# facebookresearch/dpr-scale

Hardware: NVIDIA H100
Metric: query+ctx pairs/sec (BERT-base, seq128) (higher is better)
Workload: dtype bf16

## Files before the change

dpr_scale_b200/csrc/gemm_wgmma.cu:

```cuda
#include <cstdlib>
#include <vector>
#include "common.cuh"
#include "dprb_internal.h"

namespace dprb {

namespace {

constexpr int BLOCK_M = 128;
constexpr int BLOCK_N = 256;
constexpr int BLOCK_K = 64;
constexpr int STAGES = 3;
constexpr int A_TILE_BYTES = BLOCK_M * BLOCK_K * 2;
constexpr int B_TILE_BYTES = BLOCK_N * BLOCK_K * 2;
constexpr int STAGE_BYTES = A_TILE_BYTES + B_TILE_BYTES;
constexpr int NUM_CONSUMERS = 2;
constexpr int NUM_THREADS = (NUM_CONSUMERS + 1) * 128;
constexpr int WG_ROWS = BLOCK_M / NUM_CONSUMERS;
constexpr int SUB_COLS = 64;
constexpr int SUB_BYTES = WG_ROWS * SUB_COLS * 2;
constexpr int STG_BYTES = WG_ROWS * BLOCK_N * 2;
constexpr int SMEM_BYTES = STAGES * STAGE_BYTES + NUM_CONSUMERS * STG_BYTES + 1024  + 128 ;
static_assert(SMEM_BYTES <= 227 * 1024, "ring + staging must fit one CTA per SM");
constexpr int PRODUCER_REGS = 40, CONSUMER_REGS = 232;
static_assert(128 * PRODUCER_REGS + NUM_CONSUMERS * 128 * CONSUMER_REGS <= 65536, "register file");

struct GemmParams {
  int M, N, K;
  int num_m_blocks, num_n_blocks;
  int k_blocks_total, k_blocks_per_split, splits;
  int units;
  int epilogue;
  void* D;
  long long ldd;
  const float* bias;
  int has_aux;
  int has_out2;
  float alpha;
  float* colsum;
  Drop drop;
  int aux_f16, out_f16;
  int save_pre;
};

struct Unit {
  int m0, n0, kb0, kb1;
};
__device__ __forceinline__ Unit unit_at(const GemmParams& p, int u) {
  const int tiles = p.num_m_blocks * p.num_n_blocks;
  const int tile = u % tiles, split = u / tiles;
  Unit w;
  w.m0 = (tile / p.num_n_blocks) * BLOCK_M;
  w.n0 = (tile % p.num_n_blocks) * BLOCK_N;
  w.kb0 = split * p.k_blocks_per_split;
  w.kb1 = min(w.kb0 + p.k_blocks_per_split, p.k_blocks_total);
  return w;
}

__device__ __forceinline__ void red_add_v2_f32(float* p, float a, float b) {
  asm volatile("red.global.add.v2.f32 [%0], {%1, %2};" ::"l"(p), "f"(a), "f"(b) : "memory");
}
__device__ __forceinline__ void wg_bar(int wg) { asm volatile("bar.sync %0, 128;" ::"r"(wg + 1) : "memory"); }

template <int A_MN, int B_MN, int F16>
__device__ __forceinline__ void mma_kblock(float (&acc)[128], uint32_t sa, uint32_t sb, int accumulate_first) {
  const uint64_t da = make_wgmma_desc_sw128(sa, A_MN ? BLOCK_K * 128 : 16, 1024);
  const uint64_t db = make_wgmma_desc_sw128(sb, B_MN ? BLOCK_K * 128 : 16, 1024);
  constexpr uint32_t A_KSTEP = (A_MN ? 16 * 128 : 32) >> 4;
  constexpr uint32_t B_KSTEP = (B_MN ? 16 * 128 : 32) >> 4;
#pragma unroll
  for (int k = 0; k < BLOCK_K / 16; ++k) {
    const int accum = (k > 0 || accumulate_first) ? 1 : 0;
    if (F16) wgmma_m64n256_ss_f16<A_MN, B_MN>(acc, da + k * A_KSTEP, db + k * B_KSTEP, accum);
    else wgmma_m64n256_ss_bf16<A_MN, B_MN>(acc, da + k * A_KSTEP, db + k * B_KSTEP, accum);
  }
}

__device__ __forceinline__ uint32_t pack_out(float a, float b, bool f16) { return f16 ? pack_f16x2(a, b) : pack_bf16x2(a, b); }

__device__ __forceinline__ uint32_t slab_base(const uint8_t* stg, int lr, int q) {
  return smem_u32(stg) + lr * 128 + ((lr & 7) << 4) + 4 * q;
}
__device__ __forceinline__ uint32_t slab_pair(uint32_t base, int c, int h) {
  return (base ^ ((c & 7) << 4)) + (c >> 3) * SUB_BYTES + h * 8 * 128;
}
__device__ __forceinline__ void sts32(uint32_t a, uint32_t v) { asm volatile("st.shared.b32 [%0], %1;" ::"r"(a), "r"(v)); }
__device__ __forceinline__ uint32_t lds32(uint32_t a) {
  uint32_t v;
  asm volatile("ld.shared.b32 %0, [%1];" : "=r"(v) : "r"(a));
  return v;
}
__device__ __forceinline__ int slab_boxes(int row0, int n0, int M, int N) {
  return row0 < M ? min(BLOCK_N / SUB_COLS, (N - n0 + SUB_COLS - 1) / SUB_COLS) : 0;
}
__device__ __forceinline__ void slab_tma_store(const CUtensorMap* m, const uint8_t* stg, int row0, int n0, int M, int N) {
  const int boxes = slab_boxes(row0, n0, M, N);
  for (int s = 0; s < boxes; ++s) tma_store_2d(m, smem_u32(stg + s * SUB_BYTES), n0 + s * SUB_COLS, row0);
  tma_store_commit();
}

template <bool ATOMIC>
__device__ __forceinline__ void epilogue_f32(const GemmParams& p, const float (&acc)[128], int row0, int n0, int lr, int q) {
#pragma unroll
  for (int h = 0; h < 2; ++h) {
    const int row = row0 + lr + 8 * h;
    if (row >= p.M) continue;
    float* drow = reinterpret_cast<float*>(p.D) + (long long)row * p.ldd;
#pragma unroll
    for (int c = 0; c < 32; ++c) {
      const int col = n0 + 8 * c + 2 * q;
      const float x = acc[4 * c + 2 * h] * p.alpha, y = acc[4 * c + 2 * h + 1] * p.alpha;
      if (ATOMIC) {
        if (col + 1 < p.N) red_add_v2_f32(drow + col, x, y);
        else if (col < p.N) atomicAdd(drow + col, x);
      } else {
        if (col < p.N) drow[col] = x + (p.bias != nullptr ? __ldg(p.bias + col) : 0.f);
        if (col + 1 < p.N) drow[col + 1] = y + (p.bias != nullptr ? __ldg(p.bias + col + 1) : 0.f);
      }
    }
  }
}

template <int EP, bool DROP, bool COLSUM>
__device__ __forceinline__ void epilogue16(const GemmParams& p, float (&acc)[128], uint32_t slab, int row0, int n0, int lr,
                                           int q, int lane) {
  const bool out_f16 = p.out_f16 != 0, aux_f16 = p.aux_f16 != 0;
#pragma unroll
  for (int c = 0; c < 32; ++c) {
    const int col = n0 + 8 * c + 2 * q;
    float2 b = make_float2(0.f, 0.f);
    if (p.bias != nullptr) {
      if (col + 1 < p.N) b = __ldg(reinterpret_cast<const float2*>(p.bias + col));
      else if (col < p.N) b.x = __ldg(p.bias + col);
    }
    float cs0 = 0.f, cs1 = 0.f;
#pragma unroll
    for (int h = 0; h < 2; ++h) {
      const int row = row0 + lr + 8 * h;
      const uint32_t sp = slab_pair(slab, c, h);
      float2 v = ffma2(make_float2(acc[4 * c + 2 * h], acc[4 * c + 2 * h + 1]), make_float2(p.alpha, p.alpha), b);
      if constexpr (EP == DPRB_EPI_BIAS_GELU) {
        float2 g, d;
        gelu_and_grad2(v, g, d);
        if (p.save_pre) d = v;
        sts32(sp, pack_bf16x2(g.x, g.y));
        acc[4 * c + 2 * h] = d.x;
        acc[4 * c + 2 * h + 1] = d.y;
        continue;
      }
      if constexpr (DROP) {
        float m0f, m1f;
        p.drop.mul2((uint32_t)row, (uint32_t)col, m0f, m1f);
        v.x *= m0f; v.y *= m1f;
      }
      if constexpr (EP == DPRB_EPI_BIAS_RESIDUAL) {
        const float2 a = unpack_16x2(lds32(sp), aux_f16);
        v.x += a.x; v.y += a.y;
      } else if constexpr (EP == DPRB_EPI_DGELU) {
        const float2 a = unpack_bf16x2(lds32(sp));
        v.x *= a.x; v.y *= a.y;
      } else if constexpr (EP == DPRB_EPI_DGELU_PRE) {
        float2 g, d;
        gelu_and_grad2(unpack_bf16x2(lds32(sp)), g, d);
        v.x *= d.x; v.y *= d.y;
      }
      const uint32_t o = pack_out(v.x, v.y, out_f16);
      sts32(sp, o);
      if (COLSUM && row < p.M && col < p.N) {
        const float2 f = unpack_bf16x2(o);
        cs0 += f.x;
        if (col + 1 < p.N) cs1 += f.y;
      }
    }
    if (COLSUM) {
#pragma unroll
      for (int o = 4; o < 32; o <<= 1) {
        cs0 += __shfl_xor_sync(0xFFFFFFFFu, cs0, o);
        cs1 += __shfl_xor_sync(0xFFFFFFFFu, cs1, o);
      }
      if (lane < 4) {
        if (col < p.N) atomicAdd(p.colsum + col, cs0);
        if (col + 1 < p.N) atomicAdd(p.colsum + col + 1, cs1);
      }
    }
  }
}

template <int A_MN, int B_MN, int F16>
__global__ void __launch_bounds__(NUM_THREADS, 1)
gemm_bf16_kernel(const __grid_constant__ CUtensorMap tmap_a, const __grid_constant__ CUtensorMap tmap_b,
                 const __grid_constant__ CUtensorMap tmap_d, const __grid_constant__ CUtensorMap tmap_aux,
                 const __grid_constant__ CUtensorMap tmap_out2, const GemmParams p) {
  extern __shared__ uint8_t smem_raw[];
  uint8_t* smem = align1024(smem_raw);
  uint8_t* staging = smem + STAGES * STAGE_BYTES;
  uint64_t* full_bar = reinterpret_cast<uint64_t*>(staging + NUM_CONSUMERS * STG_BYTES);
  uint64_t* empty_bar = full_bar + STAGES;
  uint64_t* aux_full = empty_bar + STAGES;
  uint64_t* slab_empty = aux_full + NUM_CONSUMERS;

  const int warp = threadIdx.x >> 5;
  const int lane = threadIdx.x & 31;
  const bool out16 = p.epilogue != DPRB_EPI_F32_ATOMIC_ADD && p.epilogue != DPRB_EPI_F32_STORE;

  if (threadIdx.x == 0) {
    tma_prefetch_desc(&tmap_a);
    tma_prefetch_desc(&tmap_b);
    if (out16) tma_prefetch_desc(&tmap_d);
    if (p.has_aux) tma_prefetch_desc(&tmap_aux);
    if (p.has_out2) tma_prefetch_desc(&tmap_out2);
    for (int i = 0; i < STAGES; ++i) {
      mbar_init(&full_bar[i], 1);
      mbar_init(&empty_bar[i], NUM_CONSUMERS * 4);
    }
    for (int i = 0; i < NUM_CONSUMERS; ++i) {
      mbar_init(&aux_full[i], 1);
      mbar_init(&slab_empty[i], 1);
    }
    fence_barrier_init();
  }
  __syncthreads();

  if (warp < 4) {
    asm volatile("setmaxnreg.dec.sync.aligned.u32 %0;" ::"n"(PRODUCER_REGS));
    if (warp == 0 && lane == 0) {
      int stage = 0;
      uint32_t phase = 0, uphase = 0;
      for (int u = blockIdx.x; u < p.units; u += gridDim.x, uphase ^= 1) {
        const Unit w = unit_at(p, u);
        const int aux_kb = min(w.kb0 + 2, w.kb1 - 1);
        for (int kb = w.kb0; kb < w.kb1; ++kb) {
          mbar_wait(&empty_bar[stage], phase ^ 1);
          mbar_arrive_expect_tx(&full_bar[stage], STAGE_BYTES);
          uint8_t* sa = smem + stage * STAGE_BYTES;
          uint8_t* sb = sa + A_TILE_BYTES;
          if (A_MN == 0) {
            tma_load_2d(sa, &tmap_a, &full_bar[stage], kb * BLOCK_K, w.m0);
          } else {
#pragma unroll
            for (int i = 0; i < BLOCK_M / 64; ++i) tma_load_2d(sa + i * (BLOCK_K * 128), &tmap_a, &full_bar[stage], w.m0 + i * 64, kb * BLOCK_K);
          }
          if (B_MN == 0) {
            tma_load_2d(sb, &tmap_b, &full_bar[stage], kb * BLOCK_K, w.n0);
          } else {
#pragma unroll
            for (int i = 0; i < BLOCK_N / 64; ++i) tma_load_2d(sb + i * (BLOCK_K * 128), &tmap_b, &full_bar[stage], w.n0 + i * 64, kb * BLOCK_K);
          }
          if (++stage == STAGES) { stage = 0; phase ^= 1; }
          if (p.has_aux && kb == aux_kb) {
            for (int g = 0; g < NUM_CONSUMERS; ++g) {
              const int row0 = w.m0 + g * WG_ROWS;
              const int boxes = slab_boxes(row0, w.n0, p.M, p.N);
              uint8_t* slab = staging + g * STG_BYTES;
              mbar_wait(&slab_empty[g], uphase);
              mbar_arrive_expect_tx(&aux_full[g], boxes * SUB_BYTES);
              for (int s = 0; s < boxes; ++s)
                tma_load_2d(slab + s * SUB_BYTES, &tmap_aux, &aux_full[g], w.n0 + s * SUB_COLS, row0);
            }
          }
        }
      }
    }
    return;
  }

  asm volatile("setmaxnreg.inc.sync.aligned.u32 %0;" ::"n"(CONSUMER_REGS));
  const int wg = (warp >> 2) - 1;
  const int t = threadIdx.x - 128 * (wg + 1);
  uint8_t* stg = staging + wg * STG_BYTES;
  const uint32_t a_off = (uint32_t)wg * (A_MN ? BLOCK_K * 128 : 64 * 128);
  const int q = lane & 3;
  const int lr = (warp & 3) * 16 + (lane >> 2);
  const uint32_t slab = slab_base(stg, lr, q);
  const int ep = p.epilogue;

  float acc[128];
  int stage = 0;
  uint32_t phase = 0, uphase = 0;
  for (int u = blockIdx.x; u < p.units; u += gridDim.x, uphase ^= 1) {
    const Unit w = unit_at(p, u);
    {
      int prev = -1;
      const int release_kb = min(w.kb0 + 1, w.kb1 - 1);
      for (int kb = w.kb0; kb < w.kb1; ++kb) {
        mbar_wait(&full_bar[stage], phase);
        const uint32_t sa = smem_u32(smem + stage * STAGE_BYTES) + a_off;
        const uint32_t sb = smem_u32(smem + stage * STAGE_BYTES + A_TILE_BYTES);
        wgmma_fence();
        mma_kblock<A_MN, B_MN, F16>(acc, sa, sb, kb > w.kb0);
        wgmma_commit();
        wgmma_wait<1>();
        if (prev >= 0) {
          __syncwarp();
          if (lane == 0) mbar_arrive(&empty_bar[prev]);
        }
        if (p.has_aux && kb == release_kb && t == 0) {
          tma_store_wait_read();
          mbar_arrive(&slab_empty[wg]);
        }
        prev = stage;
        if (++stage == STAGES) { stage = 0; phase ^= 1; }
      }
      wgmma_wait<0>();
      __syncwarp();
      if (lane == 0) mbar_arrive(&empty_bar[prev]);
    }

    const int row0 = w.m0 + wg * WG_ROWS;
    switch (ep) {
      case DPRB_EPI_F32_ATOMIC_ADD: epilogue_f32<true>(p, acc, row0, w.n0, lr, q); continue;
      case DPRB_EPI_F32_STORE: epilogue_f32<false>(p, acc, row0, w.n0, lr, q); continue;
      default: break;
    }
    if (p.has_aux) mbar_wait(&aux_full[wg], uphase);
    else if (t == 0) tma_store_wait_read();
    wg_bar(wg);
    const bool cs = p.colsum != nullptr, drop = p.drop.on();
    switch (ep) {
      case DPRB_EPI_BIAS:
        if (cs) epilogue16<DPRB_EPI_BIAS, false, true>(p, acc, slab, row0, w.n0, lr, q, lane);
        else epilogue16<DPRB_EPI_BIAS, false, false>(p, acc, slab, row0, w.n0, lr, q, lane);
        break;
      case DPRB_EPI_BIAS_GELU: epilogue16<DPRB_EPI_BIAS_GELU, false, false>(p, acc, slab, row0, w.n0, lr, q, lane); break;
      case DPRB_EPI_BIAS_RESIDUAL:
        if (drop) {
          if (cs) epilogue16<DPRB_EPI_BIAS_RESIDUAL, true, true>(p, acc, slab, row0, w.n0, lr, q, lane);
          else epilogue16<DPRB_EPI_BIAS_RESIDUAL, true, false>(p, acc, slab, row0, w.n0, lr, q, lane);
        } else {
          if (cs) epilogue16<DPRB_EPI_BIAS_RESIDUAL, false, true>(p, acc, slab, row0, w.n0, lr, q, lane);
          else epilogue16<DPRB_EPI_BIAS_RESIDUAL, false, false>(p, acc, slab, row0, w.n0, lr, q, lane);
        }
        break;
      case DPRB_EPI_DGELU:
        if (cs) epilogue16<DPRB_EPI_DGELU, false, true>(p, acc, slab, row0, w.n0, lr, q, lane);
        else epilogue16<DPRB_EPI_DGELU, false, false>(p, acc, slab, row0, w.n0, lr, q, lane);
        break;
      default:
        if (cs) epilogue16<DPRB_EPI_DGELU_PRE, false, true>(p, acc, slab, row0, w.n0, lr, q, lane);
        else epilogue16<DPRB_EPI_DGELU_PRE, false, false>(p, acc, slab, row0, w.n0, lr, q, lane);
        break;
    }
    fence_proxy_async_smem();
    wg_bar(wg);
    if (t == 0) slab_tma_store(&tmap_d, stg, row0, w.n0, p.M, p.N);
    if (p.has_out2) {
      if (t == 0) tma_store_wait_read();
      wg_bar(wg);
#pragma unroll
      for (int c = 0; c < 32; ++c)
#pragma unroll
        for (int h = 0; h < 2; ++h)
          sts32(slab_pair(slab, c, h), pack_bf16x2(acc[4 * c + 2 * h], acc[4 * c + 2 * h + 1]));
      fence_proxy_async_smem();
      wg_bar(wg);
      if (t == 0) slab_tma_store(&tmap_out2, stg, row0, w.n0, p.M, p.N);
    }
  }
  if (t == 0) tma_store_wait_all();
}

int make_tmap(CUtensorMap* out, const void* base, long long rows, long long cols, long long ld, int box_rows) {
  DPRB_REQUIRE((reinterpret_cast<uintptr_t>(base) & 15) == 0, "gemm operand base %p not 16-byte aligned", base);
  DPRB_REQUIRE((ld * 2) % 16 == 0, "gemm operand leading dimension %lld not a multiple of 8 elements", ld);
  const cuuint64_t dims[2] = {(cuuint64_t)cols, (cuuint64_t)rows};
  const cuuint64_t strides[1] = {(cuuint64_t)ld * 2};
  const cuuint32_t box[2] = {64u, (cuuint32_t)box_rows};
  return encode_tmap(out, "gemm", CU_TENSOR_MAP_DATA_TYPE_BFLOAT16, 2, base, dims, strides, box,
                     CU_TENSOR_MAP_L2_PROMOTION_L2_256B);
}

struct GemmProfile {
  bool enabled = false;
  std::vector<cudaEvent_t> ev;
  std::vector<double> flops;
  size_t used = 0;
};
GemmProfile g_prof;

int choose_splits(int tiles, int k_blocks, int sms) {
  int best = 1;
  double best_cost = 1e30;
  for (int s = 1; s <= 32; ++s) {
    if (k_blocks / s < 4 && s > 1) break;
    const int rounds = (tiles * s + sms - 1) / sms;
    const double cost = (double)rounds * ((k_blocks + s - 1) / s + 4);
    if (cost < best_cost - 1e-9) { best_cost = cost; best = s; }
  }
  return best;
}

}

int gemm_bf16(const void* A, const void* B, void* D, int M, int N, int K, long long lda, long long ldb,
              long long ldd, int a_mn_major, int b_mn_major, int epilogue, const float* bias, const void* aux,
              long long ld_aux, void* out2, float alpha, int splits, float* colsum, float dropout_p,
              unsigned long long drop_site_seed, cudaStream_t stream) {
  DPRB_REQUIRE(M > 0 && N > 0 && K > 0, "gemm: empty problem M=%d N=%d K=%d", M, N, K);
  const int dt_flags = epilogue & ~0xFF;
  epilogue &= 0xFF;
  const int a_f16 = (dt_flags & DPRB_GEMM_A_F16) != 0, b_f16 = (dt_flags & DPRB_GEMM_B_F16) != 0;
  const int aux_f16 = (dt_flags & DPRB_GEMM_AUX_F16) != 0, out_f16 = (dt_flags & DPRB_GEMM_OUT_F16) != 0;
  DPRB_REQUIRE(epilogue >= 0 && epilogue < DPRB_EPI_COUNT, "gemm: bad epilogue %d", epilogue);
  DPRB_REQUIRE(!(aux_f16 || out_f16) || epilogue == DPRB_EPI_BIAS || epilogue == DPRB_EPI_BIAS_RESIDUAL,
               "gemm: fp16 aux / output is implemented for the BIAS and BIAS_RESIDUAL epilogues only");
  DPRB_REQUIRE(a_f16 == b_f16, "gemm: wgmma takes no fp16 x bf16 operand pair: give "
               "DPRB_GEMM_A_F16 and DPRB_GEMM_B_F16 together or not at all");
  DPRB_REQUIRE(!out_f16 || colsum == nullptr, "gemm: colsum reads a bf16 slab (not available with fp16 output)");
  const bool f32_out = (epilogue == DPRB_EPI_F32_ATOMIC_ADD || epilogue == DPRB_EPI_F32_STORE);
  DPRB_REQUIRE(f32_out || (ldd % 8 == 0 && (reinterpret_cast<uintptr_t>(D) & 15) == 0),
               "gemm: bf16 output must be 16-byte aligned with ldd %% 8 == 0 (ldd=%lld)", ldd);
  DPRB_REQUIRE(!f32_out || (ldd % 4 == 0 && (reinterpret_cast<uintptr_t>(D) & 15) == 0),
               "gemm: fp32 output must be 16-byte aligned with ldd %% 4 == 0 (ldd=%lld)", ldd);
  const bool has_aux = epilogue == DPRB_EPI_BIAS_RESIDUAL || epilogue == DPRB_EPI_DGELU || epilogue == DPRB_EPI_DGELU_PRE;
  if (has_aux)
    DPRB_REQUIRE(aux != nullptr && ld_aux % 8 == 0 && (reinterpret_cast<uintptr_t>(aux) & 15) == 0,
                 "gemm: epilogue %d needs a 16-byte aligned aux with ld %% 8 == 0", epilogue);
  if (bias != nullptr) DPRB_REQUIRE((reinterpret_cast<uintptr_t>(bias) & 15) == 0, "gemm: bias not 16B aligned");

  DPRB_REQUIRE(colsum == nullptr || (!f32_out && epilogue != DPRB_EPI_BIAS_GELU),
               "gemm: colsum is supported for the BIAS / BIAS_RESIDUAL / DGELU epilogues only");

  const bool has_out2 = epilogue == DPRB_EPI_BIAS_GELU && out2 != nullptr;
  if (has_out2)
    DPRB_REQUIRE((reinterpret_cast<uintptr_t>(out2) & 15) == 0, "gemm: out2 not 16-byte aligned");

  CUtensorMap ta, tb, td{}, tx{}, to2{};
  int rc;
  if (!a_mn_major) rc = make_tmap(&ta, A, M, K, lda, BLOCK_M); else rc = make_tmap(&ta, A, K, M, lda, BLOCK_K);
  if (rc) return rc;
  if (!b_mn_major) rc = make_tmap(&tb, B, N, K, ldb, BLOCK_N); else rc = make_tmap(&tb, B, K, N, ldb, BLOCK_K);
  if (rc) return rc;
  if (!f32_out && (rc = make_tmap(&td, D, M, N, ldd, WG_ROWS))) return rc;
  if (has_aux && (rc = make_tmap(&tx, aux, M, N, ld_aux, WG_ROWS))) return rc;
  if (has_out2 && (rc = make_tmap(&to2, out2, M, N, ldd, WG_ROWS))) return rc;

  GemmParams p;
  p.M = M; p.N = N; p.K = K;
  p.num_m_blocks = (M + BLOCK_M - 1) / BLOCK_M;
  p.num_n_blocks = (N + BLOCK_N - 1) / BLOCK_N;
  p.k_blocks_total = (K + BLOCK_K - 1) / BLOCK_K;
  DPRB_NUM_SMS(sms);
  const int tiles = p.num_m_blocks * p.num_n_blocks;
  if (epilogue != DPRB_EPI_F32_ATOMIC_ADD) splits = 1;
  else if (splits <= 0) splits = choose_splits(tiles, p.k_blocks_total, sms);
  if (splits > p.k_blocks_total) splits = p.k_blocks_total;
  p.k_blocks_per_split = (p.k_blocks_total + splits - 1) / splits;
  p.splits = (p.k_blocks_total + p.k_blocks_per_split - 1) / p.k_blocks_per_split;
  p.epilogue = epilogue;
  p.D = D; p.ldd = ldd; p.bias = bias; p.has_aux = has_aux; p.has_out2 = has_out2; p.alpha = alpha;
  p.colsum = colsum;
  p.aux_f16 = aux_f16; p.out_f16 = out_f16;
  p.save_pre = (dt_flags & DPRB_GEMM_SAVE_PRE) != 0;
  p.drop = drop_from_site(epilogue == DPRB_EPI_BIAS_RESIDUAL ? dropout_p : 0.f, drop_site_seed);

  p.units = tiles * p.splits;
  const int grid = p.units < sms ? p.units : sms;
  static bool attr_set = false;
  if (!attr_set) {
#define DPRB_SET_ATTR(...) DPRB_CHECK_CUDA(cudaFuncSetAttribute(__VA_ARGS__, cudaFuncAttributeMaxDynamicSharedMemorySize, SMEM_BYTES));
    DPRB_SET_ATTR(gemm_bf16_kernel<0, 0, 0>) DPRB_SET_ATTR(gemm_bf16_kernel<0, 1, 0>)
    DPRB_SET_ATTR(gemm_bf16_kernel<1, 0, 0>) DPRB_SET_ATTR(gemm_bf16_kernel<1, 1, 0>)
    DPRB_SET_ATTR(gemm_bf16_kernel<0, 0, 1>) DPRB_SET_ATTR(gemm_bf16_kernel<0, 1, 1>)
    DPRB_SET_ATTR(gemm_bf16_kernel<1, 0, 1>) DPRB_SET_ATTR(gemm_bf16_kernel<1, 1, 1>)
#undef DPRB_SET_ATTR
    attr_set = true;
  }
  auto launch = [&](auto kern) -> int {
    const bool prof = g_prof.enabled && g_prof.used + 2 <= g_prof.ev.size();
    if (prof) DPRB_CHECK_CUDA(cudaEventRecord(g_prof.ev[g_prof.used], stream));
    kern<<<grid, NUM_THREADS, SMEM_BYTES, stream>>>(ta, tb, td, tx, to2, p);
    DPRB_LAUNCH_CHECK();
    if (prof) {
      DPRB_CHECK_CUDA(cudaEventRecord(g_prof.ev[g_prof.used + 1], stream));
      g_prof.flops.push_back(2.0 * (double)M * (double)N * (double)K);
      g_prof.used += 2;
    }
    return 0;
  };
  const int key = (a_mn_major ? 4 : 0) | (b_mn_major ? 2 : 0) | (a_f16 ? 1 : 0);
  switch (key) {
    case 0: return launch(gemm_bf16_kernel<0, 0, 0>);
    case 1: return launch(gemm_bf16_kernel<0, 0, 1>);
    case 2: return launch(gemm_bf16_kernel<0, 1, 0>);
    case 3: return launch(gemm_bf16_kernel<0, 1, 1>);
    case 4: return launch(gemm_bf16_kernel<1, 0, 0>);
    case 5: return launch(gemm_bf16_kernel<1, 0, 1>);
    case 6: return launch(gemm_bf16_kernel<1, 1, 0>);
    default: return launch(gemm_bf16_kernel<1, 1, 1>);
  }
}

int gemm_profile_enable(int enable, int max_launches) {
  if (enable) {
    const size_t want = (size_t)max_launches * 2;
    while (g_prof.ev.size() < want) {
      cudaEvent_t e;
      DPRB_CHECK_CUDA(cudaEventCreate(&e));
      g_prof.ev.push_back(e);
    }
    g_prof.used = 0;
    g_prof.flops.clear();
  }
  g_prof.enabled = enable != 0;
  return 0;
}

int gemm_profile_read(double* total_ms, double* total_flops, long long* launches) {
  double ms = 0.0, fl = 0.0;
  for (size_t i = 0; i + 1 < g_prof.used; i += 2) {
    DPRB_CHECK_CUDA(cudaEventSynchronize(g_prof.ev[i + 1]));
    float t = 0.f;
    DPRB_CHECK_CUDA(cudaEventElapsedTime(&t, g_prof.ev[i], g_prof.ev[i + 1]));
    ms += t;
    fl += g_prof.flops[i / 2];
  }
  if (total_ms) *total_ms = ms;
  if (total_flops) *total_flops = fl;
  if (launches) *launches = (long long)(g_prof.used / 2);
  return 0;
}

}
```

Baseline: 764.1.

## Add ping-pong warpgroup GEMM kernel for short-K bf16-output GEMMs

Adds a ping-pong schedule GEMM in which the two consumer warpgroups each own a whole 128x128 tile and alternate mainloops through named barriers. This lets one warpgroup's epilogue overlap the other's MMA. It uses a 5-stage ring and prefetches the residual aux tile by TMA during the mainloop, and is selected for non-fp32 outputs with K up to 1024. The dropout-residual math is also fused into an FMA, with a rounding split between row halves. In exchange it uses narrower N tiles, which means more B reloads, and adds more synchronisation complexity.

Result: faster. 781.4 (median of 6 runs) (+2.3%).

```diff
diff --git a/dpr_scale_b200/csrc/gemm_pingpong_sched.h b/dpr_scale_b200/csrc/gemm_pingpong_sched.h
--- /dev/null
+++ b/dpr_scale_b200/csrc/gemm_pingpong_sched.h
@@ -0,0 +1,43 @@
+#pragma once
+
+#if defined(__CUDACC__)
+#define DPRB_HD __host__ __device__ __forceinline__
+#else
+#define DPRB_HD inline
+#endif
+
+namespace dprb {
+namespace pingpong {
+
+constexpr int STAGES = 5;
+constexpr int CONSUMERS = 2;
+
+DPRB_HD int cta_units(int units, int grid, int cta) { return cta < units ? (units - cta + grid - 1) / grid : 0; }
+DPRB_HD int unit_of(int grid, int cta, int i) { return cta + i * grid; }
+DPRB_HD int owner(int i) { return i % CONSUMERS; }
+DPRB_HD int owner_seq(int i) { return i / CONSUMERS; }
+DPRB_HD int first_unit(int wg) { return wg; }
+DPRB_HD int next_unit(int i) { return i + CONSUMERS; }
+
+struct Slot {
+  int stage;
+  unsigned phase;
+};
+DPRB_HD Slot slot(int i, int kb, int kb_per_unit) {
+  const int f = i * kb_per_unit + kb;
+  Slot s;
+  s.stage = f % STAGES;
+  s.phase = (unsigned)((f / STAGES) & 1);
+  return s;
+}
+
+DPRB_HD bool waits_turn(int i) { return i > 0; }
+DPRB_HD bool passes_turn(int i, int n) { return i + 1 < n; }
+DPRB_HD int turn_barrier(int wg) { return 3 + wg; }
+
+DPRB_HD int release_kb(int kb_per_unit) { return kb_per_unit > 1 ? 1 : 0; }
+DPRB_HD int aux_kb(int kb_per_unit) { return kb_per_unit > 2 ? 2 : kb_per_unit - 1; }
+DPRB_HD unsigned slab_phase(int i) { return (unsigned)(owner_seq(i) & 1); }
+
+}
+}
diff --git a/dpr_scale_b200/csrc/gemm_wgmma.cu b/dpr_scale_b200/csrc/gemm_wgmma.cu
--- a/dpr_scale_b200/csrc/gemm_wgmma.cu
+++ b/dpr_scale_b200/csrc/gemm_wgmma.cu
@@ -2,6 +2,7 @@
 #include <vector>
 #include "common.cuh"
 #include "dprb_internal.h"
+#include "gemm_pingpong_sched.h"
 
 namespace dprb {
 
@@ -121,6 +122,15 @@
   }
 }
 
+template <bool DROP>
+__device__ __forceinline__ float2 drop_residual(const Drop& d, float2 v, float2 a, uint32_t row, uint32_t col, int h) {
+  if constexpr (!DROP) return make_float2(v.x + a.x, v.y + a.y);
+  float m0, m1;
+  d.mul2(row, col, m0, m1);
+  if (h == 0) return make_float2(__fmaf_rn(v.x, m0, a.x), __fmaf_rn(v.y, m1, a.y));
+  return make_float2(__fadd_rn(__fmul_rn(v.x, m0), a.x), __fadd_rn(__fmul_rn(v.y, m1), a.y));
+}
+
 template <int EP, bool DROP, bool COLSUM>
 __device__ __forceinline__ void epilogue16(const GemmParams& p, float (&acc)[128], uint32_t slab, int row0, int n0, int lr,
                                            int q, int lane) {
@@ -148,14 +158,9 @@
         acc[4 * c + 2 * h + 1] = d.y;
         continue;
       }
-      if constexpr (DROP) {
-        float m0f, m1f;
-        p.drop.mul2((uint32_t)row, (uint32_t)col, m0f, m1f);
-        v.x *= m0f; v.y *= m1f;
-      }
       if constexpr (EP == DPRB_EPI_BIAS_RESIDUAL) {
         const float2 a = unpack_16x2(lds32(sp), aux_f16);
-        v.x += a.x; v.y += a.y;
+        v = drop_residual<DROP>(p.drop, v, a, (uint32_t)row, (uint32_t)col, h);
       } else if constexpr (EP == DPRB_EPI_DGELU) {
         const float2 a = unpack_bf16x2(lds32(sp));
         v.x *= a.x; v.y *= a.y;
@@ -357,6 +362,304 @@
     }
   }
   if (t == 0) tma_store_wait_all();
+}
+
+namespace pingpong_kernel {
+
+constexpr int PP_BLOCK_N = 128;
+constexpr int PP_STAGES = pingpong::STAGES;
+constexpr int PP_STAGE_BYTES = A_TILE_BYTES + PP_BLOCK_N * BLOCK_K * 2;
+constexpr int SUB_COLS = 64;
+constexpr int PP_SUB_BYTES = BLOCK_M * SUB_COLS * 2;
+constexpr int PP_STG_BYTES = BLOCK_M * PP_BLOCK_N * 2;
+constexpr int PP_SMEM_BYTES = PP_STAGES * PP_STAGE_BYTES + NUM_CONSUMERS * PP_STG_BYTES + 1024 + 128;
+static_assert(PP_SMEM_BYTES <= 227 * 1024, "ring + staging must fit one CTA per SM");
+constexpr int MAX_KBLOCKS = 16;
+static_assert(NUM_CONSUMERS == pingpong::CONSUMERS, "one ping-pong turn per consumer warpgroup");
+
+__device__ __forceinline__ Unit unit_at128(const GemmParams& p, int u) {
+  Unit w;
+  w.m0 = (u / p.num_n_blocks) * BLOCK_M;
+  w.n0 = (u % p.num_n_blocks) * PP_BLOCK_N;
+  w.kb0 = 0;
+  w.kb1 = p.k_blocks_total;
+  return w;
+}
+__device__ __forceinline__ void named_bar_arrive(int id, int n) { asm volatile("bar.arrive %0, %1;" ::"r"(id), "r"(n) : "memory"); }
+
+template <int MN>
+__device__ __forceinline__ uint64_t operand_desc(uint32_t s) { return make_wgmma_desc_sw128(s, MN ? BLOCK_K * 128 : 16, 1024); }
+template <int MN>
+constexpr uint32_t kstep() { return (MN ? 16 * 128 : 32) >> 4; }
+template <int MN>
+constexpr uint32_t half_off() { return MN ? BLOCK_K * 128 : 64 * 128; }
+
+template <int A_MN, int B_MN, int F16>
+__device__ __forceinline__ void mma_kblock_128(float (&acc)[2][64], uint32_t sa, uint32_t sb, int accumulate_first) {
+  const uint64_t da0 = operand_desc<A_MN>(sa), da1 = operand_desc<A_MN>(sa + half_off<A_MN>());
+  const uint64_t db = operand_desc<B_MN>(sb);
+#pragma unroll
+  for (int k = 0; k < BLOCK_K / 16; ++k) {
+    const int accum = (k > 0 || accumulate_first) ? 1 : 0;
+    if (F16) {
+      wgmma_m64n128_ss_f16<A_MN, B_MN>(acc[0], da0 + k * kstep<A_MN>(), db + k * kstep<B_MN>(), accum);
+      wgmma_m64n128_ss_f16<A_MN, B_MN>(acc[1], da1 + k * kstep<A_MN>(), db + k * kstep<B_MN>(), accum);
+    } else {
+      wgmma_m64n128_ss_bf16<A_MN, B_MN>(acc[0], da0 + k * kstep<A_MN>(), db + k * kstep<B_MN>(), accum);
+      wgmma_m64n128_ss_bf16<A_MN, B_MN>(acc[1], da1 + k * kstep<A_MN>(), db + k * kstep<B_MN>(), accum);
+    }
+  }
+}
+
+template <int A_MN, int B_MN, int BN>
+__device__ __forceinline__ void load_kblock(uint8_t* sa, const CUtensorMap* ta, const CUtensorMap* tb, uint64_t* bar,
+                                            int m0, int n0, int kb) {
+  uint8_t* sb = sa + A_TILE_BYTES;
+  if (A_MN == 0) {
+    tma_load_2d(sa, ta, bar, kb * BLOCK_K, m0);
+  } else {
+#pragma unroll
+    for (int i = 0; i < BLOCK_M / 64; ++i) tma_load_2d(sa + i * (BLOCK_K * 128), ta, bar, m0 + i * 64, kb * BLOCK_K);
+  }
+  if (B_MN == 0) {
+    tma_load_2d(sb, tb, bar, kb * BLOCK_K, n0);
+  } else {
+#pragma unroll
+    for (int i = 0; i < BN / 64; ++i) tma_load_2d(sb + i * (BLOCK_K * 128), tb, bar, n0 + i * 64, kb * BLOCK_K);
+  }
+}
+
+__device__ __forceinline__ uint32_t slab_base(const uint8_t* stg, int lr, int q) {
+  return smem_u32(stg) + lr * 128 + ((lr & 7) << 4) + 4 * q;
+}
+__device__ __forceinline__ uint32_t slab_pair(uint32_t base, int hm, int c, int h) {
+  return (base ^ ((c & 7) << 4)) + (c >> 3) * PP_SUB_BYTES + hm * 64 * 128 + h * 8 * 128;
+}
+__device__ __forceinline__ int slab_boxes(int n0, int N) { return min(PP_BLOCK_N / SUB_COLS, (N - n0 + SUB_COLS - 1) / SUB_COLS); }
+__device__ __forceinline__ void slab_tma_store(const CUtensorMap* m, const uint8_t* stg, int m0, int n0, int N) {
+  const int boxes = slab_boxes(n0, N);
+  for (int s = 0; s < boxes; ++s) tma_store_2d(m, smem_u32(stg + s * PP_SUB_BYTES), n0 + s * SUB_COLS, m0);
+  tma_store_commit();
+}
+
+template <int EP, bool DROP, bool COLSUM>
+__device__ __forceinline__ void epilogue16(const GemmParams& p, float (&acc)[2][64], uint32_t slab, int m0, int n0, int lr,
+                                           int q, int lane) {
+  const bool out_f16 = p.out_f16 != 0, aux_f16 = p.aux_f16 != 0;
+#pragma unroll
+  for (int c = 0; c < 16; ++c) {
+    const int col = n0 + 8 * c + 2 * q;
+    float2 b = make_float2(0.f, 0.f);
+    if (p.bias != nullptr) {
+      if (col + 1 < p.N) b = __ldg(reinterpret_cast<const float2*>(p.bias + col));
+      else if (col < p.N) b.x = __ldg(p.bias + col);
+    }
+    float cs0 = 0.f, cs1 = 0.f;
+#pragma unroll
+    for (int hm = 0; hm < 2; ++hm) {
+#pragma unroll
+      for (int h = 0; h < 2; ++h) {
+        const int row = m0 + 64 * hm + lr + 8 * h;
+        const uint32_t sp = slab_pair(slab, hm, c, h);
+        float& a0 = acc[hm][4 * c + 2 * h];
+        float& a1 = acc[hm][4 * c + 2 * h + 1];
+        float2 v = ffma2(make_float2(a0, a1), make_float2(p.alpha, p.alpha), b);
+        if constexpr (EP == DPRB_EPI_BIAS_GELU) {
+          float2 g, d;
+          gelu_and_grad2(v, g, d);
+          if (p.save_pre) d = v;
+          sts32(sp, pack_bf16x2(g.x, g.y));
+          a0 = d.x;
+          a1 = d.y;
+          continue;
+        }
+        if constexpr (EP == DPRB_EPI_BIAS_RESIDUAL) {
+          const float2 a = unpack_16x2(lds32(sp), aux_f16);
+          v = drop_residual<DROP>(p.drop, v, a, (uint32_t)row, (uint32_t)col, h);
+        } else if constexpr (EP == DPRB_EPI_DGELU) {
+          const float2 a = unpack_bf16x2(lds32(sp));
+          v.x *= a.x; v.y *= a.y;
+        } else if constexpr (EP == DPRB_EPI_DGELU_PRE) {
+          float2 g, d;
+          gelu_and_grad2(unpack_bf16x2(lds32(sp)), g, d);
+          v.x *= d.x; v.y *= d.y;
+        }
+        const uint32_t o = pack_out(v.x, v.y, out_f16);
+        sts32(sp, o);
+        if (COLSUM && row < p.M && col < p.N) {
+          const float2 f = unpack_bf16x2(o);
+          cs0 += f.x;
+          if (col + 1 < p.N) cs1 += f.y;
+        }
+      }
+    }
+    if (COLSUM) {
+#pragma unroll
+      for (int o = 4; o < 32; o <<= 1) {
+        cs0 += __shfl_xor_sync(0xFFFFFFFFu, cs0, o);
+        cs1 += __shfl_xor_sync(0xFFFFFFFFu, cs1, o);
+      }
+      if (lane < 4) {
+        if (col < p.N) atomicAdd(p.colsum + col, cs0);
+        if (col + 1 < p.N) atomicAdd(p.colsum + col + 1, cs1);
+      }
+    }
+  }
+}
+
+template <int A_MN, int B_MN, int F16>
+__global__ void __launch_bounds__(NUM_THREADS, 1)
+gemm_pingpong_kernel(const __grid_constant__ CUtensorMap tmap_a, const __grid_constant__ CUtensorMap tmap_b,
+                     const __grid_constant__ CUtensorMap tmap_d, const __grid_constant__ CUtensorMap tmap_aux,
+                     const __grid_constant__ CUtensorMap tmap_out2, const GemmParams p) {
+  namespace pp = pingpong;
+  extern __shared__ uint8_t smem_raw[];
+  uint8_t* smem = align1024(smem_raw);
+  uint8_t* staging = smem + PP_STAGES * PP_STAGE_BYTES;
+  uint64_t* full_bar = reinterpret_cast<uint64_t*>(staging + NUM_CONSUMERS * PP_STG_BYTES);
+  uint64_t* empty_bar = full_bar + PP_STAGES;
+  uint64_t* aux_full = empty_bar + PP_STAGES;
+  uint64_t* slab_empty = aux_full + NUM_CONSUMERS;
+
+  const int warp = threadIdx.x >> 5;
+  const int lane = threadIdx.x & 31;
+
+  if (threadIdx.x == 0) {
+    tma_prefetch_desc(&tmap_a);
+    tma_prefetch_desc(&tmap_b);
+    tma_prefetch_desc(&tmap_d);
+    if (p.has_aux) tma_prefetch_desc(&tmap_aux);
+    if (p.has_out2) tma_prefetch_desc(&tmap_out2);
+    for (int i = 0; i < PP_STAGES; ++i) {
+      mbar_init(&full_bar[i], 1);
+      mbar_init(&empty_bar[i], 4);
+    }
+    for (int i = 0; i < NUM_CONSUMERS; ++i) {
+      mbar_init(&aux_full[i], 1);
+      mbar_init(&slab_empty[i], 1);
+    }
+    fence_barrier_init();
+  }
+  __syncthreads();
+
+  if (warp < 4) {
+    asm volatile("setmaxnreg.dec.sync.aligned.u32 %0;" ::"n"(PRODUCER_REGS));
+    if (warp == 0 && lane == 0) {
+      const int kbs = p.k_blocks_total;
+      const int n = pp::cta_units(p.units, gridDim.x, blockIdx.x);
+      for (int i = 0; i < n; ++i) {
+        const Unit w = unit_at128(p, pp::unit_of(gridDim.x, blockIdx.x, i));
+        const int g = pp::owner(i);
+        for (int kb = 0; kb < kbs; ++kb) {
+          const pp::Slot s = pp::slot(i, kb, kbs);
+          mbar_wait(&empty_bar[s.stage], s.phase ^ 1);
+          mbar_arrive_expect_tx(&full_bar[s.stage], PP_STAGE_BYTES);
+          load_kblock<A_MN, B_MN, PP_BLOCK_N>(smem + s.stage * PP_STAGE_BYTES, &tmap_a, &tmap_b, &full_bar[s.stage],
+                                              w.m0, w.n0, kb);
+          if (p.has_aux && kb == pp::aux_kb(kbs)) {
+            const int boxes = slab_boxes(w.n0, p.N);
+            uint8_t* slab = staging + g * PP_STG_BYTES;
+            mbar_wait(&slab_empty[g], pp::slab_phase(i));
+            mbar_arrive_expect_tx(&aux_full[g], boxes * PP_SUB_BYTES);
+            for (int s2 = 0; s2 < boxes; ++s2)
+              tma_load_2d(slab + s2 * PP_SUB_BYTES, &tmap_aux, &aux_full[g], w.n0 + s2 * SUB_COLS, w.m0);
+          }
+        }
+      }
+    }
+    return;
+  }
+
+  asm volatile("setmaxnreg.inc.sync.aligned.u32 %0;" ::"n"(CONSUMER_REGS));
+  const int wg = (warp >> 2) - 1;
+  const int t = threadIdx.x - 128 * (wg + 1);
+  uint8_t* stg = staging + wg * PP_STG_BYTES;
+  const int q = lane & 3;
+  const int lr = (warp & 3) * 16 + (lane >> 2);
+  const uint32_t slab = slab_base(stg, lr, q);
+  const int ep = p.epilogue;
+  const int kbs = p.k_blocks_total;
+  const int n = pp::cta_units(p.units, gridDim.x, blockIdx.x);
+
+  float acc[2][64];
+  for (int i = pp::first_unit(wg); i < n; i = pp::next_unit(i)) {
+    const Unit w = unit_at128(p, pp::unit_of(gridDim.x, blockIdx.x, i));
+    if (p.has_aux && t == 0) {
+      tma_store_wait_read();
+      mbar_arrive(&slab_empty[wg]);
+    }
+    if (pp::waits_turn(i)) named_bar_sync(pp::turn_barrier(wg), 2 * 128);
+    {
+      int prev = -1;
+      for (int kb = 0; kb < kbs; ++kb) {
+        const pp::Slot s = pp::slot(i, kb, kbs);
+        mbar_wait(&full_bar[s.stage], s.phase);
+        const uint32_t sa = smem_u32(smem + s.stage * PP_STAGE_BYTES);
+        wgmma_fence();
+        mma_kblock_128<A_MN, B_MN, F16>(acc, sa, sa + A_TILE_BYTES, kb > 0);
+        wgmma_commit();
+        wgmma_wait<1>();
+        if (prev >= 0) {
+          __syncwarp();
+          if (lane == 0) mbar_arrive(&empty_bar[prev]);
+        }
+        prev = s.stage;
+      }
+      if (pp::passes_turn(i, n)) named_bar_arrive(pp::turn_barrier(pp::owner(i + 1)), 2 * 128);
+      wgmma_wait<0>();
+      __syncwarp();
+      if (lane == 0) mbar_arrive(&empty_bar[prev]);
+    }
+
+    if (p.has_aux) mbar_wait(&aux_full[wg], pp::slab_phase(i));
+    else if (t == 0) tma_store_wait_read();
+    wg_bar(wg);
+    const bool cs = p.colsum != nullptr, drop = p.drop.on();
+    switch (ep) {
+      case DPRB_EPI_BIAS:
+        if (cs) epilogue16<DPRB_EPI_BIAS, false, true>(p, acc, slab, w.m0, w.n0, lr, q, lane);
+        else epilogue16<DPRB_EPI_BIAS, false, false>(p, acc, slab, w.m0, w.n0, lr, q, lane);
+        break;
+      case DPRB_EPI_BIAS_GELU: epilogue16<DPRB_EPI_BIAS_GELU, false, false>(p, acc, slab, w.m0, w.n0, lr, q, lane); break;
+      case DPRB_EPI_BIAS_RESIDUAL:
+        if (drop) {
+          if (cs) epilogue16<DPRB_EPI_BIAS_RESIDUAL, true, true>(p, acc, slab, w.m0, w.n0, lr, q, lane);
+          else epilogue16<DPRB_EPI_BIAS_RESIDUAL, true, false>(p, acc, slab, w.m0, w.n0, lr, q, lane);
+        } else {
+          if (cs) epilogue16<DPRB_EPI_BIAS_RESIDUAL, false, true>(p, acc, slab, w.m0, w.n0, lr, q, lane);
+          else epilogue16<DPRB_EPI_BIAS_RESIDUAL, false, false>(p, acc, slab, w.m0, w.n0, lr, q, lane);
+        }
+        break;
+      case DPRB_EPI_DGELU:
+        if (cs) epilogue16<DPRB_EPI_DGELU, false, true>(p, acc, slab, w.m0, w.n0, lr, q, lane);
+        else epilogue16<DPRB_EPI_DGELU, false, false>(p, acc, slab, w.m0, w.n0, lr, q, lane);
+        break;
+      default:
+        if (cs) epilogue16<DPRB_EPI_DGELU_PRE, false, true>(p, acc, slab, w.m0, w.n0, lr, q, lane);
+        else epilogue16<DPRB_EPI_DGELU_PRE, false, false>(p, acc, slab, w.m0, w.n0, lr, q, lane);
+        break;
+    }
+    fence_proxy_async_smem();
+    wg_bar(wg);
+    if (t == 0) slab_tma_store(&tmap_d, stg, w.m0, w.n0, p.N);
+    if (p.has_out2) {
+      if (t == 0) tma_store_wait_read();
+      wg_bar(wg);
+#pragma unroll
+      for (int hm = 0; hm < 2; ++hm)
+#pragma unroll
+        for (int c = 0; c < 16; ++c)
+#pragma unroll
+          for (int h = 0; h < 2; ++h)
+            sts32(slab_pair(slab, hm, c, h), pack_bf16x2(acc[hm][4 * c + 2 * h], acc[hm][4 * c + 2 * h + 1]));
+      fence_proxy_async_smem();
+      wg_bar(wg);
+      if (t == 0) slab_tma_store(&tmap_out2, stg, w.m0, w.n0, p.N);
+    }
+  }
+  if (t == 0) tma_store_wait_all();
+}
+
 }
 
 int make_tmap(CUtensorMap* out, const void* base, long long rows, long long cols, long long ld, int box_rows) {
@@ -424,20 +727,23 @@
   if (has_out2)
     DPRB_REQUIRE((reinterpret_cast<uintptr_t>(out2) & 15) == 0, "gemm: out2 not 16-byte aligned");
 
+  const bool pingpong = !f32_out && (K + BLOCK_K - 1) / BLOCK_K <= pingpong_kernel::MAX_KBLOCKS;
+  const int block_n = pingpong ? pingpong_kernel::PP_BLOCK_N : BLOCK_N;
+  const int slab_rows = pingpong ? BLOCK_M : WG_ROWS;
   CUtensorMap ta, tb, td{}, tx{}, to2{};
   int rc;
   if (!a_mn_major) rc = make_tmap(&ta, A, M, K, lda, BLOCK_M); else rc = make_tmap(&ta, A, K, M, lda, BLOCK_K);
   if (rc) return rc;
-  if (!b_mn_major) rc = make_tmap(&tb, B, N, K, ldb, BLOCK_N); else rc = make_tmap(&tb, B, K, N, ldb, BLOCK_K);
+  if (!b_mn_major) rc = make_tmap(&tb, B, N, K, ldb, block_n); else rc = make_tmap(&tb, B, K, N, ldb, BLOCK_K);
   if (rc) return rc;
-  if (!f32_out && (rc = make_tmap(&td, D, M, N, ldd, WG_ROWS))) return rc;
-  if (has_aux && (rc = make_tmap(&tx, aux, M, N, ld_aux, WG_ROWS))) return rc;
-  if (has_out2 && (rc = make_tmap(&to2, out2, M, N, ldd, WG_ROWS))) return rc;
+  if (!f32_out && (rc = make_tmap(&td, D, M, N, ldd, slab_rows))) return rc;
+  if (has_aux && (rc = make_tmap(&tx, aux, M, N, ld_aux, slab_rows))) return rc;
+  if (has_out2 && (rc = make_tmap(&to2, out2, M, N, ldd, slab_rows))) return rc;
 
   GemmParams p;
   p.M = M; p.N = N; p.K = K;
   p.num_m_blocks = (M + BLOCK_M - 1) / BLOCK_M;
-  p.num_n_blocks = (N + BLOCK_N - 1) / BLOCK_N;
+  p.num_n_blocks = (N + block_n - 1) / block_n;
   p.k_blocks_total = (K + BLOCK_K - 1) / BLOCK_K;
   DPRB_NUM_SMS(sms);
   const int tiles = p.num_m_blocks * p.num_n_blocks;
@@ -463,12 +769,19 @@
     DPRB_SET_ATTR(gemm_bf16_kernel<0, 0, 1>) DPRB_SET_ATTR(gemm_bf16_kernel<0, 1, 1>)
     DPRB_SET_ATTR(gemm_bf16_kernel<1, 0, 1>) DPRB_SET_ATTR(gemm_bf16_kernel<1, 1, 1>)
 #undef DPRB_SET_ATTR
+    using namespace pingpong_kernel;
+#define DPRB_SET_ATTR(...) DPRB_CHECK_CUDA(cudaFuncSetAttribute(__VA_ARGS__, cudaFuncAttributeMaxDynamicSharedMemorySize, PP_SMEM_BYTES));
+    DPRB_SET_ATTR(gemm_pingpong_kernel<0, 0, 0>) DPRB_SET_ATTR(gemm_pingpong_kernel<0, 1, 0>)
+    DPRB_SET_ATTR(gemm_pingpong_kernel<1, 0, 0>) DPRB_SET_ATTR(gemm_pingpong_kernel<1, 1, 0>)
+    DPRB_SET_ATTR(gemm_pingpong_kernel<0, 0, 1>) DPRB_SET_ATTR(gemm_pingpong_kernel<0, 1, 1>)
+    DPRB_SET_ATTR(gemm_pingpong_kernel<1, 0, 1>) DPRB_SET_ATTR(gemm_pingpong_kernel<1, 1, 1>)
+#undef DPRB_SET_ATTR
     attr_set = true;
   }
   auto launch = [&](auto kern) -> int {
     const bool prof = g_prof.enabled && g_prof.used + 2 <= g_prof.ev.size();
     if (prof) DPRB_CHECK_CUDA(cudaEventRecord(g_prof.ev[g_prof.used], stream));
-    kern<<<grid, NUM_THREADS, SMEM_BYTES, stream>>>(ta, tb, td, tx, to2, p);
+    kern<<<grid, NUM_THREADS, pingpong ? pingpong_kernel::PP_SMEM_BYTES : SMEM_BYTES, stream>>>(ta, tb, td, tx, to2, p);
     DPRB_LAUNCH_CHECK();
     if (prof) {
       DPRB_CHECK_CUDA(cudaEventRecord(g_prof.ev[g_prof.used + 1], stream));
@@ -478,6 +791,19 @@
     return 0;
   };
   const int key = (a_mn_major ? 4 : 0) | (b_mn_major ? 2 : 0) | (a_f16 ? 1 : 0);
+  if (pingpong) {
+    using namespace pingpong_kernel;
+    switch (key) {
+      case 0: return launch(gemm_pingpong_kernel<0, 0, 0>);
+      case 1: return launch(gemm_pingpong_kernel<0, 0, 1>);
+      case 2: return launch(gemm_pingpong_kernel<0, 1, 0>);
+      case 3: return launch(gemm_pingpong_kernel<0, 1, 1>);
+      case 4: return launch(gemm_pingpong_kernel<1, 0, 0>);
+      case 5: return launch(gemm_pingpong_kernel<1, 0, 1>);
+      case 6: return launch(gemm_pingpong_kernel<1, 1, 0>);
+      default: return launch(gemm_pingpong_kernel<1, 1, 1>);
+    }
+  }
   switch (key) {
     case 0: return launch(gemm_bf16_kernel<0, 0, 0>);
     case 1: return launch(gemm_bf16_kernel<0, 0, 1>);
```
